# omahs/cess

Hardware: AMD Instinct MI355X
Metric: verified BLS12-381 sigs/sec (node) (higher is better)
Workload: dtype u32 (381-bit Montgomery, 14x28-bit limb products via v_mad_u64_u32)

## Files before the change

cess_amd/csrc/bls/pair_fe.hpp:

```cpp
#pragma once
#include "pair.hpp"

#if !defined(CESS_HOSTEMU)
namespace bls {

struct GlobPair {
  uint4* base;
  uint64_t stride;
  CESS_HD uint64_t at(int k, int q) const {
    const uint32_t l = lane_fresh();
    return (uint64_t)(6 * k + q + 3 * (l & 1u)) * stride + (l >> 1);
  }
  CESS_HD fph ld(int k) const {
    fph r;
#pragma unroll
    for (int q = 0; q < 3; q++) {
      const uint4 x = base[at(k, q)];
      r.v.v[4 * q] = x.x, r.v.v[4 * q + 1] = x.y, r.v.v[4 * q + 2] = x.z, r.v.v[4 * q + 3] = x.w;
    }
    return r;
  }
  CESS_HD void st(int k, const fph& a) const {
#pragma unroll
    for (int q = 0; q < 3; q++)
      base[at(k, q)] = make_uint4(a.v.v[4 * q], a.v.v[4 * q + 1], a.v.v[4 * q + 2], a.v.v[4 * q + 3]);
  }
  CESS_HD fp2 ld_full(int k) const {
    const uint32_t l = lane_fresh() >> 1;
    fp2 r;
#pragma unroll
    for (int q = 0; q < 6; q++) {
      const uint4 x = base[(uint64_t)(6 * k + q) * stride + l];
      fp& d = q < 3 ? r.c0 : r.c1;
      const int o = 4 * (q % 3);
      d.v[o] = x.x, d.v[o + 1] = x.y, d.v[o + 2] = x.z, d.v[o + 3] = x.w;
    }
    return r;
  }
  CESS_HD void st_full(int k, const fp2& a) const {
    const uint32_t l = lane_fresh() >> 1;
#pragma unroll
    for (int q = 0; q < 6; q++) {
      const fp& s = q < 3 ? a.c0 : a.c1;
      const int o = 4 * (q % 3);
      base[(uint64_t)(6 * k + q) * stride + l] = make_uint4(s.v[o], s.v[o + 1], s.v[o + 2], s.v[o + 3]);
    }
  }
};

template <class D, class S>
CESS_HD void pcopy12(const D& d, const S& s) {
#pragma unroll 1
  for (int k = 0; k < 6; k++) d.st(k, s.ld(k));
}
template <class S>
CESS_HD void pconj12(const S& f) {
#pragma unroll 1
  for (int k = 3; k < 6; k++) f.st(k, neg(f.ld(k)));
}
template <class S>
CESS_HD bool pis_one12(const S& f) {
  bool r = eq(f.ld(0).v, fph_one().v);
#pragma unroll 1
  for (int k = 1; k < 6; k++) r = r && is_zero(f.ld(k).v);
  return pair_and(r);
}
template <class A, class B>
CESS_HD bool pis_conj12(const A& a, const B& b) {
  bool r = true;
#pragma unroll 1
  for (int k = 0; k < 6; k++) r = r && eq(a.ld(k).v, k < 3 ? b.ld(k).v : neg(b.ld(k).v));
  return pair_and(r);
}

template <class LA>
CESS_HD fp6h pmul6_lr(LA&& a, const fp6h& b) {
#if CESS_PAIR_SB
  return pmul6_sb(a, b);
#endif
  const fph v0 = pmul(a(0), b.c0);
  CESS_MEMBAR();
  const fph v1 = pmul(a(1), b.c1);
  CESS_MEMBAR();
  const fph v2 = pmul(a(2), b.c2);
  CESS_MEMBAR();
  const fph c0 = add(mul_nr(sub(sub(pmul(add_nr(a(1), a(2)), add_nr(b.c1, b.c2)), v1), v2)), v0);
  CESS_MEMBAR();
  const fph c1 = add(sub(sub(pmul(add_nr(a(0), a(1)), add_nr(b.c0, b.c1)), v0), v1), mul_nr(v2));
  CESS_MEMBAR();
  const fph c2 = add(sub(sub(pmul(add_nr(a(0), a(2)), add_nr(b.c0, b.c2)), v0), v2), v1);
  return {c0, c1, c2};
}

#ifndef CESS_PAIR_FE_LOOP
#define CESS_PAIR_FE_LOOP 1
#endif
template <class S, class G>
CESS_HD void pmul12(const S& f, const G& g) {
#if CESS_PAIR_FE_LOOP
  fp6h t0;
#pragma unroll 1
  for (int it = 0; it < 3; it++) {
    fp6h b;
    if (it == 1) {
      b = add_nr(pld6(g, 0), pld6(g, 1));
    } else {
      b = pld6(g, it >> 1);
    }
    const fp6h r = pmul6_lr(
        [&](int j) {
          const int lo = it == 2 ? 3 : 0;
          const fph a = f.ld(lo + j);
          return it == 1 ? add_nr(a, f.ld(3 + j)) : a;
        },
        b);
    CESS_MEMBAR();
    if (it == 0) {
      t0 = r;
    } else if (it == 1) {
      pst6(f, 0, sub(r, t0));
    } else {
      pst6(f, 1, sub(pld6(f, 0), r));
      pst6(f, 0, add(t0, mul_v(r)));
    }
  }
#else
  fp6h t0;
  {
    const fp6h g0 = pld6(g, 0);
    t0 = pmul6_lr([&](int j) { return f.ld(j); }, g0);
  }
  CESS_MEMBAR();
  {
    fp6h gs;
    {
      const fp6h g0 = pld6(g, 0), g1 = pld6(g, 1);
      gs = add_nr(g0, g1);
    }
    const fp6h x = pmul6_lr([&](int j) { return add_nr(f.ld(j), f.ld(3 + j)); }, gs);
    CESS_MEMBAR();
    pst6(f, 0, sub(x, t0));
  }
  CESS_MEMBAR();
  fp6h t1;
  {
    const fp6h g1 = pld6(g, 1);
    t1 = pmul6_lr([&](int j) { return f.ld(3 + j); }, g1);
  }
  CESS_MEMBAR();
  pst6(f, 1, sub(pld6(f, 0), t1));
  pst6(f, 0, add(t0, mul_v(t1)));
#endif
}

template <class S>
CESS_HD fp6h psqr6(const S& f, int h) {
  const fp6h a = pld6(f, h);
  return pmul6_lr([&](int j) { return f.ld(3 * h + j); }, a);
}

template <class S>
CESS_HD void pinv12(const S& f) {
  fp6h ti;
  {
    fp6h t;
    {
      const fp6h s0 = psqr6(f, 0);
      CESS_MEMBAR();
      t = sub(s0, mul_v(psqr6(f, 1)));
    }
    CESS_MEMBAR();
    const fph c0 = sub(pmul(t.c0, t.c0), mul_nr(pmul(t.c1, t.c2)));
    CESS_MEMBAR();
    const fph c1 = sub(mul_nr(pmul(t.c2, t.c2)), pmul(t.c0, t.c1));
    CESS_MEMBAR();
    const fph c2 = sub(pmul(t.c1, t.c1), pmul(t.c0, t.c2));
    CESS_MEMBAR();
    const fph den = add(pmul(t.c0, c0), mul_nr(pdot2(t.c2, c1, t.c1, c2)));
    const fph di = pinv(den);
    CESS_MEMBAR();
    ti = {pmul(c0, di), pmul(c1, di), pmul(c2, di)};
  }
  CESS_MEMBAR();
  pst6(f, 0, pmul6_lr([&](int j) { return f.ld(j); }, ti));
  CESS_MEMBAR();
  const fp6h r1 = pmul6_lr([&](int j) { return f.ld(3 + j); }, ti);
  pst6(f, 1, {neg(r1.c0), neg(r1.c1), neg(r1.c2)});
}

CESS_HD fph pfrob_coeff(int k, int i) {
  const uint32_t hm = pair_hi_mask();
  fp r;
#pragma unroll
  for (int w = 0; w < 12; w++) r.v[w] = (c::FROB[k - 1][i][1][w] & hm) | (c::FROB[k - 1][i][0][w] & ~hm);
  return {r};
}
template <class S>
CESS_HD void pfrob12(const S& f, int k) {
#pragma unroll 1
  for (int s = 0; s < 6; s++) {
    const int i = (s % 3) * 2 + s / 3;
    fph y = f.ld(s);
    if (k & 1) y = conj(y);
    if (i) y = pmul(y, pfrob_coeff(k, i));
    f.st(s, y);
  }
}

CESS_HD void pfp4_square(fph& c0, fph& c1, const fph& a, const fph& b) {
  const fph t0 = pmul(a, b);
  CESS_MEMBAR();
  const fph t = pmul(add_nr(a, b), add_xi_nr(a, b));
  c0 = sub(sub(t, t0), mul_nr(t0));
  c1 = dbl(t0);
}
CESS_HD void pcyc_square_regs(fph (&z)[6], int n) {
#pragma unroll 1
  for (int r = 0; r < n; r++) {
    CESS_MEMBAR();
    fph t0, t1;
    pfp4_square(t0, t1, z[0], z[4]);
    z[0] = add(dbl(sub(t0, z[0])), t0);
    z[4] = add(dbl(add(t1, z[4])), t1);
    CESS_MEMBAR();
    fph t2, t3;
    pfp4_square(t0, t1, z[3], z[2]);
    CESS_MEMBAR();
    pfp4_square(t2, t3, z[1], z[5]);
    z[1] = add(dbl(sub(t0, z[1])), t0);
    z[5] = add(dbl(add(t1, z[5])), t1);
    const fph n3 = mul_nr(t3);
    z[3] = add(dbl(add(n3, z[3])), n3);
    z[2] = add(dbl(sub(t2, z[2])), t2);
  }
}
template <class S>
CESS_HD void pcyc_square_run(const S& f, int n) {
  fph z[6];
#pragma unroll
  for (int k = 0; k < 6; k++) z[k] = f.ld(k);
  pcyc_square_regs(z, n);
#pragma unroll
  for (int k = 0; k < 6; k++) f.st(k, z[k]);
}

CESS_HD void pkcyc_run(fph& z2, fph& z3, fph& z4, fph& z5, int n) {
#pragma unroll 1
  for (int r = 0; r < n; r++) {
    CESS_MEMBAR();
    fph u, v;
    {
      const fph b3 = pmul_scaled<3>(z4, z5);
      CESS_MEMBAR();
      const fph t3 = pmul_scaled<3>(add_nr(z4, z5), add_xi_nr(z4, z5));
      const fph nb3 = mul_nr(b3);
      u = sub(sub(t3, b3), nb3);
      v = dbl(nb3);
    }
    CESS_MEMBAR();
    {
      const fph b3 = pmul_scaled<3>(z2, z3);
      CESS_MEMBAR();
      const fph t3 = pmul_scaled<3>(add_nr(z2, z3), add_xi_nr(z2, z3));
      z4 = sub(sub(sub(t3, b3), mul_nr(b3)), dbl(z4));
      z5 = dbl(add(z5, b3));
    }
    CESS_MEMBAR();
    z2 = add(dbl(z2), v);
    z3 = sub(u, dbl(z3));
  }
}

CESS_HD fp2 xchg2(const fp2& a) { return {xchg(a.c0), xchg(a.c1)}; }

CESS_HD void ps_operands(const fp2& u, const fp2& w, bool hi, fp2& s, fp2& y) {
  uint32_t bn = 0, k0 = 0, k1 = 0, k2 = 0, k3 = 0;
#pragma unroll
  for (int i = 0; i < 12; i++) {
    const uint32_t z0 = hi ? u.c0.v[i] : w.c0.v[i], z1 = hi ? u.c1.v[i] : w.c1.v[i];
    const uint32_t nz1 = subc32(c::P2_RAW[i], z1, bn, &bn);
    s.c0.v[i] = addc32(u.c0.v[i], w.c0.v[i], k0, &k0);
    s.c1.v[i] = addc32(u.c1.v[i], w.c1.v[i], k1, &k1);
    y.c0.v[i] = addc32(s.c0.v[i], nz1, k2, &k2);
    y.c1.v[i] = addc32(s.c1.v[i], z0, k3, &k3);
  }
}
CESS_HD void pkcyc_run_ps(fp2& u, fp2& w, int n) {
  const bool hi = pair_hi_mask() != 0;
#pragma unroll 1
  for (int r = 0; r < n; r++) {
    CESS_MEMBAR();
    fp2 P, Q;
    {
      const fp2 b3 = mul_scaled<3>(u, w);
      CESS_MEMBAR();
      fp2 s, y;
      ps_operands(u, w, hi, s, y);
      const fp2 t3 = mul_scaled<3>(s, y);
      const fp2 nb3 = mul_nr(b3);
      P = sub(sub(t3, b3), nb3);
      Q = select(hi, b3, nb3);
    }
    CESS_MEMBAR();
    P = xchg2(P);
    Q = xchg2(Q);
    u = sub(P, dbl(u));
    w = dbl(add(w, Q));
  }
}

CESS_HD void pcyc_z1_frac(const fph& z2, const fph& z3, const fph& z4, const fph& z5, fph& num, fph& den) {
  if (is_zero(z2)) {
    num = dbl(pmul(z4, z5));
    den = z3;
  } else {
    num = sub(add(mul_nr(psqr(z5)), mul3(psqr(z4))), dbl(z3));
    den = dbl(dbl(z2));
  }
}
CESS_HD fph pcyc_z1_den(const fph& z2, const fph& z3) { return is_zero(z2) ? z3 : dbl(dbl(z2)); }
CESS_HD fph pcyc_z0(const fph& z1, const fph& z2, const fph& z3, const fph& z4, const fph& z5) {
  return add(mul_nr(add(dbl(psqr(z1)), pdot2(z2, z5, neg(mul3(z3)), z4))), fph_one());
}

template <class B, class XFn>
CESS_HD void pcyc_chain(const B& base, XFn&& X) {
  constexpr int ND = CESS_CHAIN_TAIL ? 3 : 6;
#ifndef CESS_PAIR_KCYC_PS
#define CESS_PAIR_KCYC_PS 1
#endif
#if CESS_PAIR_KCYC_PS
  {
    const bool hi = pair_hi_mask() != 0;
    const int ku = hi ? 2 : 1, kw = hi ? 3 : 5;
    fp2 u = base.ld_full(ku), w = base.ld_full(kw);
    int k = 0;
#pragma unroll 1
    for (int j = 0; j < ND; j++) {
      const int stop = j == 0 ? 16 : j == 1 ? 48 : j == 2 ? 57 : j == 3 ? 60 : j == 4 ? 62 : 63;
      pkcyc_run_ps(u, w, stop - k);
      k = stop;
      CESS_MEMBAR();
      const auto x = X(j);
      x.st_full(ku, u);
      x.st_full(kw, w);
    }
  }
#else
  {
    fph z4 = base.ld(1), z5 = base.ld(5), z2 = base.ld(3), z3 = base.ld(2);
    int k = 0;
#pragma unroll 1
    for (int j = 0; j < ND; j++) {
      const int stop = j == 0 ? 16 : j == 1 ? 48 : j == 2 ? 57 : j == 3 ? 60 : j == 4 ? 62 : 63;
      pkcyc_run(z2, z3, z4, z5, stop - k);
      k = stop;
      CESS_MEMBAR();
      const auto x = X(j);
      x.st(3, z2);
      x.st(2, z3);
      x.st(1, z4);
      x.st(5, z5);
    }
  }
#endif
  CESS_MEMBAR();
  bool degen = false;
  fph prod = fph_one();
#pragma unroll 1
  for (int j = 0; j < ND; j++) {
    const auto x = X(j);
    fph num, den;
    pcyc_z1_frac(x.ld(3), x.ld(2), x.ld(1), x.ld(5), num, den);
    const bool z = is_zero(den);
    degen = degen || z;
    x.st(4, num);
    x.st(0, prod);
    prod = pmul(prod, select(z, fph_one(), den));
    CESS_MEMBAR();
  }
  fph iv = pinv(prod);
#pragma unroll 1
  for (int j = ND - 1; j >= 0; j--) {
    const auto x = X(j);
    const fph den = pcyc_z1_den(x.ld(3), x.ld(2));
    const fph ivj = pmul(iv, x.ld(0));
    iv = pmul(iv, select(is_zero(den), fph_one(), den));
    CESS_MEMBAR();
    const fph z1 = pmul(x.ld(4), ivj);
    x.st(4, z1);
    CESS_MEMBAR();
    x.st(0, pcyc_z0(z1, x.ld(3), x.ld(2), x.ld(1), x.ld(5)));
    CESS_MEMBAR();
  }
  if (degen) {
    const auto w = X(5);
    pcopy12(w, base);
#pragma unroll 1
    for (int j = 0; j < 5; j++) {
      const int run = j == 0 ? 16 : j == 1 ? 32 : j == 2 ? 9 : j == 3 ? 3 : 2;
      pcyc_square_run(w, run);
      pcopy12(X(j), w);
    }
    pcyc_square_run(w, 1);
  }
#if CESS_CHAIN_TAIL
  else {
    fph z[6];
    {
      const auto x2 = X(2);
#pragma unroll
      for (int k = 0; k < 6; k++) z[k] = x2.ld(k);
    }
#pragma unroll 1
    for (int j = 3; j < 6; j++) {
      pcyc_square_regs(z, j == 3 ? 3 : j == 4 ? 2 : 1);
      CESS_MEMBAR();
      const auto x = X(j);
#pragma unroll
      for (int k = 0; k < 6; k++) x.st(k, z[k]);
    }
  }
#endif
}

template <class A, class SlotFn>
CESS_HD void final_exp_pair(const A& acc, const uint8_t (*prog)[2], SlotFn&& slot) {
#pragma unroll 1
  for (int pc = 0;; pc++) {
    const uint8_t op = prog[pc][0], arg = prog[pc][1];
    if (op == FE_END) break;
    switch (op) {
      case FE_LOAD: pcopy12(acc, slot(arg)); break;
      case FE_STORE: pcopy12(slot(arg), acc); break;
      case FE_MUL: pmul12(acc, slot(arg)); break;
      case FE_SQN: pcyc_square_run(acc, arg); break;
      case FE_CONJ: pconj12(acc); break;
      case FE_FROB: pfrob12(acc, arg); break;
      case FE_INV: pinv12(acc); break;
      case FE_CHAIN: pcyc_chain(slot(arg), [&](int j) { return slot(SL_X0 + j); }); break;
      default: break;
    }
    CESS_MEMBAR();
  }
}

}
#endif
```

cess_amd/csrc/bls/staged.hpp:

```cpp
#pragma once
#include "pairing.hpp"
#include "diag.hpp"

namespace bls {

#if !defined(CESS_HOSTEMU)
CESS_HD uint32_t lane_fresh() {
  uint32_t l;
  asm volatile("v_mbcnt_lo_u32_b32 %0, -1, 0\n\tv_mbcnt_hi_u32_b32 %0, -1, %0" : "=v"(l));
  return l;
}
CESS_HD uint32_t wave_first_thread() { return __builtin_amdgcn_readfirstlane(threadIdx.x & ~63u); }

struct LdsF12 {
  uint4 (*F)[256];
  uint32_t w0;
  CESS_HD fp2 ld(int k) const {
    const uint32_t t = w0 + lane_fresh();
    fp2 r;
#pragma unroll
    for (int q = 0; q < 6; q++) {
      uint4 x = F[6 * k + q][t];
      fp& d = q < 3 ? r.c0 : r.c1;
      const int o = 4 * (q % 3);
      d.v[o] = x.x, d.v[o + 1] = x.y, d.v[o + 2] = x.z, d.v[o + 3] = x.w;
    }
    return r;
  }
  CESS_HD void st(int k, const fp2& a) const {
    const uint32_t t = w0 + lane_fresh();
#pragma unroll
    for (int q = 0; q < 6; q++) {
      const fp& s = q < 3 ? a.c0 : a.c1;
      const int o = 4 * (q % 3);
      F[6 * k + q][t] = make_uint4(s.v[o], s.v[o + 1], s.v[o + 2], s.v[o + 3]);
    }
  }
};

struct GlobF12W {
  uint4* base;
  uint64_t stride;
  CESS_HD fp2 ld(int k) const {
    const uint32_t l = lane_fresh();
    fp2 r;
#pragma unroll
    for (int q = 0; q < 6; q++) {
      uint4 x = base[(uint64_t)(6 * k + q) * stride + l];
      fp& d = q < 3 ? r.c0 : r.c1;
      const int o = 4 * (q % 3);
      d.v[o] = x.x, d.v[o + 1] = x.y, d.v[o + 2] = x.z, d.v[o + 3] = x.w;
    }
    return r;
  }
  CESS_HD void st(int k, const fp2& a) const {
    const uint32_t l = lane_fresh();
#pragma unroll
    for (int q = 0; q < 6; q++) {
      const fp& s = q < 3 ? a.c0 : a.c1;
      const int o = 4 * (q % 3);
      const uint4 v = make_uint4(s.v[o], s.v[o + 1], s.v[o + 2], s.v[o + 3]);
      base[(uint64_t)(6 * k + q) * stride + l] = v;
    }
  }
};

struct GlobF12 {
  uint4* base;
  uint64_t stride;
  uint32_t i;
  CESS_HD fp2 ld(int k) const {
    fp2 r;
#pragma unroll
    for (int q = 0; q < 6; q++) {
      uint4 x = base[(uint64_t)(6 * k + q) * stride + i];
      fp& d = q < 3 ? r.c0 : r.c1;
      const int o = 4 * (q % 3);
      d.v[o] = x.x, d.v[o + 1] = x.y, d.v[o + 2] = x.z, d.v[o + 3] = x.w;
    }
    return r;
  }
  CESS_HD void st(int k, const fp2& a) const {
#pragma unroll
    for (int q = 0; q < 6; q++) {
      const fp& s = q < 3 ? a.c0 : a.c1;
      const int o = 4 * (q % 3);
      base[(uint64_t)(6 * k + q) * stride + i] = make_uint4(s.v[o], s.v[o + 1], s.v[o + 2], s.v[o + 3]);
    }
  }
};
#endif

struct ArrF12 {
  fp12* p;
  CESS_HD fp2 ld(int k) const { return (&p->c0.c0)[k]; }
  CESS_HD void st(int k, const fp2& a) const { (&p->c0.c0)[k] = a; }
};

template <class S>
CESS_HD fp6 ld6(const S& s, int h) {
  return {s.ld(3 * h), s.ld(3 * h + 1), s.ld(3 * h + 2)};
}
template <class S>
CESS_HD void st6(const S& s, int h, const fp6& a) {
  s.st(3 * h, a.c0);
  s.st(3 * h + 1, a.c1);
  s.st(3 * h + 2, a.c2);
}
template <class D, class S>
CESS_HD void copy12(const D& d, const S& s) {
#pragma unroll 1
  for (int k = 0; k < 6; k++) d.st(k, s.ld(k));
}
template <class S>
CESS_HD void set_one12(const S& s) {
  s.st(0, fp2_one());
#pragma unroll 1
  for (int k = 1; k < 6; k++) s.st(k, fp2_zero());
}
template <class S>
CESS_HD void conj12(const S& s) {
#pragma unroll 1
  for (int k = 3; k < 6; k++) s.st(k, neg(s.ld(k)));
}
template <class S>
CESS_HD bool is_one12(const S& s) {
  bool r = eq(s.ld(0), fp2_one());
#pragma unroll 1
  for (int k = 1; k < 6; k++) r = r && is_zero(s.ld(k));
  return r;
}

template <class A, class B>
CESS_HD bool is_conj12(const A& a, const B& b) {
  bool r = true;
#pragma unroll 1
  for (int k = 0; k < 6; k++) r = r && eq(a.ld(k), k < 3 ? b.ld(k) : neg(b.ld(k)));
  return r;
}

#ifndef CESS_SQR12_LOOP
#define CESS_SQR12_LOOP 0
#endif
#ifndef CESS_MUL014_LOOP
#define CESS_MUL014_LOOP 0
#endif
template <class S>
CESS_HD void sqr12(const S& f) {
#if CESS_SQR12_LOOP
  fp6 ab;
#pragma unroll 1
  for (int it = 0; it < 2; it++) {
    fp6 x, y;
    {
      const fp6 a0 = ld6(f, 0), a1 = ld6(f, 1);
      if (it) {
        x = add_nr(a0, a1);
        y = add_nr(a0, mul_v(a1));
      } else {
        x = a0;
        y = a1;
      }
    }
    const fp6 r = mul(x, y);
    CESS_MEMBAR();
    if (it) {
      st6(f, 0, sub(sub(r, ab), mul_v(ab)));
      st6(f, 1, dbl(ab));
    } else {
      ab = r;
    }
  }
#else
  fp6 ab;
  {
    fp6 a0 = ld6(f, 0), a1 = ld6(f, 1);
    ab = mul(a0, a1);
  }
  CESS_MEMBAR();
  fp6 x;
  {
    fp6 a0 = ld6(f, 0), a1 = ld6(f, 1);
    x = mul(add_nr(a0, a1), add_nr(a0, mul_v(a1)));
  }
  st6(f, 0, sub(sub(x, ab), mul_v(ab)));
  st6(f, 1, dbl(ab));
#endif
}

template <class S>
CESS_HD fp6 mul_by_01_dot(const S& f, int h, const fp2& b0, const fp2& b1, const fp2& xb1) {
  fp6 r;
  r.c0 = dot2(f.ld(3 * h), b0, f.ld(3 * h + 2), xb1);
  CESS_MEMBAR();
  r.c1 = dot2(f.ld(3 * h), b1, f.ld(3 * h + 1), b0);
  CESS_MEMBAR();
  r.c2 = dot2(f.ld(3 * h + 1), b1, f.ld(3 * h + 2), b0);
  return r;
}

template <class S>
CESS_HD void mul014(const S& f, const fp2& c0, const fp2& c1, const fp2& c4) {
#if CESS_MUL014_LOOP
  fp6 bb = mul_by_1(ld6(f, 1), c4);
  CESS_MEMBAR();
  fp6 aa;
  const fp2 d = add(c1, c4);
#pragma unroll 1
  for (int it = 0; it < 2; it++) {
    const fp2 b1 = it ? d : c1;
    const fp6 r = mul_by_01_dot(f, it, c0, b1, mul_nr(b1));
    CESS_MEMBAR();
    if (it) {
      st6(f, 1, sub(r, add(aa, bb)));
    } else {
      aa = r;
      {
        fp6 s = add(ld6(f, 0), ld6(f, 1));
        st6(f, 1, s);
      }
      st6(f, 0, add(mul_v(bb), aa));
    }
  }
#else
  fp6 bb = mul_by_1(ld6(f, 1), c4);
  CESS_MEMBAR();
  fp6 aa = mul_by_01_dot(f, 0, c0, c1, mul_nr(c1));
  CESS_MEMBAR();
  {
    fp6 s = add(ld6(f, 0), ld6(f, 1));
    st6(f, 1, s);
  }
  st6(f, 0, add(mul_v(bb), aa));
  fp6 u = add(aa, bb);
  CESS_MEMBAR();
  const fp2 d = add(c1, c4);
  fp6 t = mul_by_01_dot(f, 1, c0, d, mul_nr(d));
  st6(f, 1, sub(t, u));
#endif
}

CESS_HD fp6 mul_by_01_one(const fp6& a, const fp2& b1) {
#if CESS_MUL2
  fp2 p2, p0;
  mul2(a.c2, b1, a.c0, b1, p2, p0);
  return {add(a.c0, mul_nr(p2)), add(a.c1, p0), add(a.c2, mul(a.c1, b1))};
#else
  return {add(a.c0, mul_nr(mul(a.c2, b1))), add(a.c1, mul(a.c0, b1)), add(a.c2, mul(a.c1, b1))};
#endif
}

template <class S>
CESS_HD void mul014_one(const S& f, const fp2& c1, const fp2& c4) {
#if CESS_MUL014_LOOP
  fp6 bb = mul_by_1(ld6(f, 1), c4);
  CESS_MEMBAR();
  fp6 aa;
  const fp2 d = add(c1, c4);
#pragma unroll 1
  for (int it = 0; it < 2; it++) {
    const fp6 r = mul_by_01_one(ld6(f, it), it ? d : c1);
    CESS_MEMBAR();
    if (it) {
      st6(f, 1, sub(r, add(aa, bb)));
    } else {
      aa = r;
      {
        fp6 s = add(ld6(f, 0), ld6(f, 1));
        st6(f, 1, s);
      }
      st6(f, 0, add(mul_v(bb), aa));
    }
  }
#else
  fp6 bb = mul_by_1(ld6(f, 1), c4);
  CESS_MEMBAR();
  fp6 aa = mul_by_01_one(ld6(f, 0), c1);
  CESS_MEMBAR();
  {
    fp6 s = add(ld6(f, 0), ld6(f, 1));
    st6(f, 1, s);
  }
  st6(f, 0, add(mul_v(bb), aa));
  fp6 u = add(aa, bb);
  CESS_MEMBAR();
  fp6 t = mul_by_01_one(ld6(f, 1), add(c1, c4));
  st6(f, 1, sub(t, u));
#endif
}

template <class S, class G>
CESS_HD void mul12(const S& f, const G& g) {
  fp6 t0, t1;
  t0 = mul(ld6(f, 0), ld6(g, 0));
  CESS_MEMBAR();
  t1 = mul(ld6(f, 1), ld6(g, 1));
  CESS_MEMBAR();
  fp6 x = mul(add_nr(ld6(f, 0), ld6(f, 1)), add_nr(ld6(g, 0), ld6(g, 1)));
  st6(f, 1, sub(sub(x, t0), t1));
  st6(f, 0, add(t0, mul_v(t1)));
}

#ifndef CESS_FE_PF
#define CESS_FE_PF 0
#endif
template <class LA, class LB, class SK>
CESS_HD void mul6_stream(LA&& a, LB&& b, SK&& sink) {
#if CESS_FE_PF
  fp2 pa = a(0), pb = b(0);
  fp2 qa = a(1), qb = b(1);
  const fp2 v0 = mul(pa, pb);
  CESS_MEMBAR();
  pa = a(2), pb = b(2);
  const fp2 v1 = mul(qa, qb);
  CESS_MEMBAR();
  const fp2 v2 = mul(pa, pb);
  CESS_MEMBAR();
#else
  const fp2 v0 = mul(a(0), b(0));
  CESS_MEMBAR();
  const fp2 v1 = mul(a(1), b(1));
  CESS_MEMBAR();
  const fp2 v2 = mul(a(2), b(2));
  CESS_MEMBAR();
#endif
  sink(0, add(mul_nr(sub(sub(mul(add_nr(a(1), a(2)), add_nr(b(1), b(2))), v1), v2)), v0));
  CESS_MEMBAR();
  sink(1, add(sub(sub(mul(add_nr(a(0), a(1)), add_nr(b(0), b(1))), v0), v1), mul_nr(v2)));
  CESS_MEMBAR();
  sink(2, add(sub(sub(mul(add_nr(a(0), a(2)), add_nr(b(0), b(2))), v0), v2), v1));
  CESS_MEMBAR();
}

template <class D, class S, class G, class T>
CESS_HD void mul12_stream(const D& d, const S& f, const G& g, const T& t) {
  mul6_stream([&](int j) { return f.ld(j); }, [&](int j) { return g.ld(j); },
              [&](int j, const fp2& v) { t.st(j, v); });
  mul6_stream([&](int j) { return f.ld(3 + j); }, [&](int j) { return g.ld(3 + j); },
              [&](int j, const fp2& v) { d.st(3 + j, v); });
  d.st(0, add(t.ld(0), mul_nr(d.ld(5))));
  d.st(1, add(t.ld(1), d.ld(3)));
  d.st(2, add(t.ld(2), d.ld(4)));
  CESS_MEMBAR();
  mul6_stream([&](int j) { return add_nr(f.ld(j), f.ld(3 + j)); },
              [&](int j) { return add_nr(g.ld(j), g.ld(3 + j)); },
              [&](int j, const fp2& x) { d.st(3 + j, sub(sub(x, t.ld(j)), d.ld(3 + j))); });
}

#ifndef CESS_FE_APARK
#define CESS_FE_APARK 1
#endif
template <class D, class S, class G, class T, class P>
CESS_HD void mul12_stream_ap(const D& d, const S& f, const G& g, const T& t, const P& pk) {
#pragma unroll 1
  for (int j = 0; j < 3; j++) pk.st(j, f.ld(j));
  CESS_MEMBAR();
  mul6_stream([&](int j) { return pk.ld(j); }, [&](int j) { return g.ld(j); },
              [&](int j, const fp2& v) { t.st(j, v); });
  CESS_MEMBAR();
#pragma unroll 1
  for (int j = 0; j < 3; j++) pk.st(j, f.ld(3 + j));
  CESS_MEMBAR();
  mul6_stream([&](int j) { return pk.ld(j); }, [&](int j) { return g.ld(3 + j); },
              [&](int j, const fp2& v) { d.st(3 + j, v); });
  d.st(0, add(t.ld(0), mul_nr(d.ld(5))));
  d.st(1, add(t.ld(1), d.ld(3)));
  d.st(2, add(t.ld(2), d.ld(4)));
  CESS_MEMBAR();
#pragma unroll 1
  for (int j = 0; j < 3; j++) pk.st(j, add_nr(f.ld(j), f.ld(3 + j)));
  CESS_MEMBAR();
  mul6_stream([&](int j) { return pk.ld(j); }, [&](int j) { return add_nr(g.ld(j), g.ld(3 + j)); },
              [&](int j, const fp2& x) { d.st(3 + j, sub(sub(x, t.ld(j)), d.ld(3 + j))); });
}

template <class S>
CESS_HD void cycsq12(const S& f) {
  {
    fp2 z0 = f.ld(0), z1 = f.ld(4), t0, t1;
    fp4_square(t0, t1, z0, z1);
    f.st(0, add(dbl(sub(t0, z0)), t0));
    f.st(4, add(dbl(add(t1, z1)), t1));
  }
  CESS_MEMBAR();
  fp2 t0, t1, t2, t3;
  fp4_square(t0, t1, f.ld(3), f.ld(2));
  fp4_square(t2, t3, f.ld(1), f.ld(5));
  f.st(1, add(dbl(sub(t0, f.ld(1))), t0));
  f.st(5, add(dbl(add(t1, f.ld(5))), t1));
  fp2 n3 = mul_nr(t3);
  f.st(3, add(dbl(add(n3, f.ld(3))), n3));
  f.st(2, add(dbl(sub(t2, f.ld(2))), t2));
}

template <class S>
CESS_HD void frob12(const S& f, int k) {
#pragma unroll 1
  for (int s = 0; s < 6; s++) {
    const int i = (s % 3) * 2 + s / 3;
    fp2 y = f.ld(s);
    if (k & 1) y = conj(y);
    if (i) y = mul(y, frob_coeff(k, i));
    f.st(s, y);
  }
}

template <class S>
CESS_HD void inv12(const S& f) {
  fp6 t;
  {
    fp6 a0 = ld6(f, 0), a1 = ld6(f, 1);
    t = sub(sqr(a0), mul_v(sqr(a1)));
  }
  t = inv(t);
  CESS_MEMBAR();
  fp6 a0 = ld6(f, 0);
  st6(f, 0, mul(a0, t));
  fp6 a1 = ld6(f, 1);
  st6(f, 1, neg(mul(a1, t)));
}

template <class D, class S, class T>
CESS_HD void inv12_stream(const D& d, const S& f, const T& t) {
  mul6_stream([&](int j) { return f.ld(j); }, [&](int j) { return f.ld(j); }, [&](int j, const fp2& v) { d.st(j, v); });
  mul6_stream([&](int j) { return f.ld(3 + j); }, [&](int j) { return f.ld(3 + j); },
              [&](int j, const fp2& v) { d.st(3 + j, v); });
  t.st(0, sub(d.ld(0), mul_nr(d.ld(5))));
  t.st(1, sub(d.ld(1), d.ld(3)));
  t.st(2, sub(d.ld(2), d.ld(4)));
  CESS_MEMBAR();
  d.st(0, sub(sqr(t.ld(0)), mul_nr(mul(t.ld(1), t.ld(2)))));
  CESS_MEMBAR();
  d.st(1, sub(mul_nr(sqr(t.ld(2))), mul(t.ld(0), t.ld(1))));
  CESS_MEMBAR();
  d.st(2, sub(sqr(t.ld(1)), mul(t.ld(0), t.ld(2))));
  CESS_MEMBAR();
  const fp2 den = inv(add(mul(t.ld(0), d.ld(0)), mul_nr(add(mul(t.ld(2), d.ld(1)), mul(t.ld(1), d.ld(2))))));
  CESS_MEMBAR();
#pragma unroll 1
  for (int j = 0; j < 3; j++) t.st(j, mul(d.ld(j), den));
  CESS_MEMBAR();
  mul6_stream([&](int j) { return f.ld(j); }, [&](int j) { return t.ld(j); }, [&](int j, const fp2& v) { d.st(j, v); });
  mul6_stream([&](int j) { return f.ld(3 + j); }, [&](int j) { return t.ld(j); },
              [&](int j, const fp2& v) { d.st(3 + j, neg(v)); });
}

enum FeOp : uint8_t { FE_LOAD, FE_STORE, FE_MUL, FE_SQN, FE_CONJ, FE_FROB, FE_INV, FE_CHAIN, FE_END };
enum FeSlot : uint8_t { SL_F = 0, SL_M, SL_T0, SL_T1, SL_T3, SL_T4, SL_T5, SL_T6,
                        SL_X0, SL_X1, SL_X2, SL_X3, SL_X4, SL_X5, SL_TM, SL_N };

#define CESS_FE_CYCEXP(s) \
  {FE_CHAIN, s}, {FE_LOAD, SL_X5}, {FE_MUL, SL_X4}, {FE_MUL, SL_X3}, {FE_MUL, SL_X2}, {FE_MUL, SL_X1}, \
      {FE_MUL, SL_X0}, {FE_CONJ, 0}

#define CESS_FE_BODY                                                                                              \
  {FE_LOAD, SL_F}, {FE_CONJ, 0}, {FE_STORE, SL_T0}, {FE_LOAD, SL_F}, {FE_INV, 0}, {FE_MUL, SL_T0},                 \
      {FE_STORE, SL_T0}, {FE_FROB, 2}, {FE_MUL, SL_T0}, {FE_STORE, SL_M},                                          \
       {FE_SQN, 1}, {FE_CONJ, 0}, {FE_STORE, SL_T1},                                     \
       CESS_FE_CYCEXP(SL_M), {FE_STORE, SL_T3},                                                      \
       {FE_SQN, 1}, {FE_STORE, SL_T4},                                                          \
       {FE_LOAD, SL_T1}, {FE_MUL, SL_T3}, {FE_STORE, SL_T5},                                     \
       CESS_FE_CYCEXP(SL_T5), {FE_STORE, SL_T1},                                                    \
       CESS_FE_CYCEXP(SL_T1), {FE_STORE, SL_T0},                                                    \
       CESS_FE_CYCEXP(SL_T0), {FE_MUL, SL_T4}, {FE_STORE, SL_T6},                             \
       CESS_FE_CYCEXP(SL_T6), {FE_STORE, SL_T4},                                                    \
       {FE_LOAD, SL_T5}, {FE_CONJ, 0}, {FE_MUL, SL_M}, {FE_MUL, SL_T4},              \
      {FE_STORE, SL_T4},                                                                                           \
       {FE_LOAD, SL_T1}, {FE_MUL, SL_M}, {FE_FROB, 3}, {FE_STORE, SL_T1},                 \
       {FE_LOAD, SL_M}, {FE_CONJ, 0}, {FE_MUL, SL_T6}, {FE_FROB, 1},              \
      {FE_STORE, SL_T6},                                                                                           \
       {FE_LOAD, SL_T3}, {FE_MUL, SL_T0}, {FE_FROB, 2}, {FE_MUL, SL_T1},  \
      {FE_MUL, SL_T6}
#define CESS_FE_PROGRAM CESS_FE_BODY, {FE_MUL, SL_T4}, {FE_END, 0}
#define CESS_FE_PROGRAM_VERIFY CESS_FE_BODY, {FE_END, 0}

template <class A, class P>
CESS_HD void cyc_square_run(const A& acc, const P& pk, int n) {
  pk.st(0, acc.ld(0));
  pk.st(1, acc.ld(4));
  fp2 z2 = acc.ld(3), z3 = acc.ld(2);
#pragma unroll 1
  for (int r = 0; r < n; r++) {
    CESS_MEMBAR();
    {
      const fp2 a = pk.ld(0), b = pk.ld(1);
      fp2 t0, t1;
      fp4_square(t0, t1, a, b);
      pk.st(0, add(dbl(sub(t0, a)), t0));
      pk.st(1, add(dbl(add(t1, b)), t1));
    }
    CESS_MEMBAR();
    fp2 u0;
    {
      fp2 u1;
      fp4_square(u0, u1, acc.ld(1), acc.ld(5));
      pk.st(2, u1);
    }
    CESS_MEMBAR();
    {
      fp2 t0, t1;
      fp4_square(t0, t1, z2, z3);
      acc.st(1, add(dbl(sub(t0, acc.ld(1))), t0));
      acc.st(5, add(dbl(add(t1, acc.ld(5))), t1));
    }
    CESS_MEMBAR();
    const fp2 n3 = mul_nr(pk.ld(2));
    z2 = add(dbl(add(n3, z2)), n3);
    z3 = add(dbl(sub(u0, z3)), u0);
  }
  CESS_MEMBAR();
  acc.st(0, pk.ld(0));
  acc.st(4, pk.ld(1));
  acc.st(3, z2);
  acc.st(2, z3);
}

#ifndef CESS_KCYC_LOOP
#define CESS_KCYC_LOOP 0
#endif
template <class P>
CESS_HD void kcyc_run(const P& pk, fp2& z2, fp2& z3, int n) {
#if CESS_KCYC_LOOP
#pragma unroll 1
  for (int r = 0; r < n; r++) {
    fp2 u, v;
#pragma unroll 1
    for (int h = 0; h < 2; h++) {
      CESS_MEMBAR();
      fp2 x, y;
      if (h) {
        x = z2;
        y = z3;
      } else {
        x = pk.ld(0);
        y = pk.ld(1);
      }
      const fp2 b3 = mul_scaled<3>(x, y);
      CESS_MEMBAR();
      const fp2 t3 = mul_scaled<3>(add_nr(x, y), add_xi_nr(x, y));
      const fp2 nb3 = mul_nr(b3);
      const fp2 w = sub(sub(t3, b3), nb3);
      if (h) {
        pk.st(0, sub(w, dbl(pk.ld(0))));
        pk.st(1, dbl(add(pk.ld(1), b3)));
      } else {
        u = w;
        v = dbl(nb3);
      }
    }
    CESS_MEMBAR();
    z2 = add(dbl(z2), v);
    z3 = sub(u, dbl(z3));
  }
#else
#pragma unroll 1
  for (int r = 0; r < n; r++) {
    CESS_MEMBAR();
    fp2 u, v;
    {
      const fp2 b3 = mul_scaled<3>(pk.ld(0), pk.ld(1));
      CESS_MEMBAR();
      const fp2 t3 = mul_scaled<3>(add_nr(pk.ld(0), pk.ld(1)), add_xi_nr(pk.ld(0), pk.ld(1)));
      const fp2 nb3 = mul_nr(b3);
      u = sub(sub(t3, b3), nb3);
      v = dbl(nb3);
    }
    CESS_MEMBAR();
    {
      const fp2 b3 = mul_scaled<3>(z2, z3);
      CESS_MEMBAR();
      const fp2 t3 = mul_scaled<3>(add_nr(z2, z3), add_xi_nr(z2, z3));
      pk.st(0, sub(sub(sub(t3, b3), mul_nr(b3)), dbl(pk.ld(0))));
      pk.st(1, dbl(add(pk.ld(1), b3)));
    }
    CESS_MEMBAR();
    z2 = add(dbl(z2), v);
    z3 = sub(u, dbl(z3));
  }
#endif
}

CESS_HD void cyc_z1_frac(const fp2& z2, const fp2& z3, const fp2& z4, const fp2& z5, fp2& num, fp2& den) {
  num = sub(add(mul_nr(sqr(z5)), mul3(sqr(z4))), dbl(z3));
  den = dbl(dbl(z2));
  if (is_zero(z2)) {
    num = dbl(mul(z4, z5));
    den = z3;
  }
}
CESS_HD fp2 cyc_z1_den(const fp2& z2, const fp2& z3) { return is_zero(z2) ? z3 : dbl(dbl(z2)); }
CESS_HD fp2 cyc_z0(const fp2& z1, const fp2& z2, const fp2& z3, const fp2& z4, const fp2& z5) {
  return add(mul_nr(add(dbl(sqr(z1)), dot2(z2, z5, neg(mul3(z3)), z4))), fp2_one());
}

#ifndef CESS_CHAIN_TAIL
#define CESS_CHAIN_TAIL 1
#endif
template <class B, class XFn, class P, class DG = NoDiag>
CESS_HD void cyc_chain(const B& base, XFn&& X, const P& pk, DG* dg = nullptr) {
  constexpr int ND = CESS_CHAIN_TAIL ? 3 : 6;
  {
    pk.st(0, base.ld(1));
    pk.st(1, base.ld(5));
    fp2 z2 = base.ld(3), z3 = base.ld(2);
    int k = 0;
#pragma unroll 1
    for (int j = 0; j < ND; j++) {
      const int stop = j == 0 ? 16 : j == 1 ? 48 : j == 2 ? 57 : j == 3 ? 60 : j == 4 ? 62 : 63;
      if (dg) dg->template mark<0>();
      kcyc_run(pk, z2, z3, stop - k);
      if (dg) dg->template mark<3>();
      k = stop;
      CESS_MEMBAR();
      const auto x = X(j);
      x.st(3, z2);
      x.st(2, z3);
      x.st(1, pk.ld(0));
      x.st(5, pk.ld(1));
    }
  }
  CESS_MEMBAR();
  bool degen = false;
  fp2 prod = fp2_one();
#pragma unroll 1
  for (int j = 0; j < ND; j++) {
    const auto x = X(j);
    fp2 num, den;
    cyc_z1_frac(x.ld(3), x.ld(2), x.ld(1), x.ld(5), num, den);
    const bool z = is_zero(den);
    degen = degen || z;
    x.st(4, num);
    x.st(0, prod);
    prod = mul(prod, select(z, fp2_one(), den));
    CESS_MEMBAR();
  }
  fp2 iv = inv(prod);
#pragma unroll 1
  for (int j = ND - 1; j >= 0; j--) {
    const auto x = X(j);
    const fp2 den = cyc_z1_den(x.ld(3), x.ld(2));
    const fp2 ivj = mul(iv, x.ld(0));
    iv = mul(iv, select(is_zero(den), fp2_one(), den));
    CESS_MEMBAR();
    const fp2 z1 = mul(x.ld(4), ivj);
    x.st(4, z1);
    CESS_MEMBAR();
    x.st(0, cyc_z0(z1, x.ld(3), x.ld(2), x.ld(1), x.ld(5)));
    CESS_MEMBAR();
  }
  if (degen) {
    const auto w = X(5);
    copy12(w, base);
#pragma unroll 1
    for (int j = 0; j < 5; j++) {
      const int run = j == 0 ? 16 : j == 1 ? 32 : j == 2 ? 9 : j == 3 ? 3 : 2;
      cyc_square_run(w, pk, run);
      copy12(X(j), w);
    }
    cyc_square_run(w, pk, 1);
  }
#if CESS_CHAIN_TAIL
  else {
#pragma unroll 1
    for (int j = 3; j < 6; j++) {
      copy12(X(j), X(j - 1));
      cyc_square_run(X(j), pk, j == 3 ? 3 : j == 4 ? 2 : 1);
    }
  }
#endif
  if (dg) dg->template mark<4>();
}

template <class A, class SlotFn, class P, class DG = NoDiag>
CESS_HD int final_exp_staged(const A& acc0, const A& acc1, const uint8_t (*prog)[2], SlotFn&& slot, const P& pk,
                             DG* dg = nullptr) {
  int cur = 0;
#pragma unroll 1
  for (int pc = 0;; pc++) {
    const uint8_t op = prog[pc][0], arg = prog[pc][1];
    if (op == FE_END) break;
    const A& acc = cur ? acc1 : acc0;
    switch (op) {
      case FE_LOAD: copy12(acc, slot(arg)); break;
      case FE_STORE: copy12(slot(arg), acc); break;
      case FE_MUL:
#if CESS_FE_APARK
        mul12_stream_ap(cur ? acc0 : acc1, acc, slot(arg), slot(SL_TM), pk);
#else
        mul12_stream(cur ? acc0 : acc1, acc, slot(arg), pk);
#endif
        cur ^= 1;
        if (dg) dg->template mark<1>();
        break;
      case FE_SQN: cyc_square_run(acc, pk, arg); break;
      case FE_CONJ: conj12(acc); break;
      case FE_FROB: frob12(acc, arg); break;
      case FE_INV:
        inv12_stream(cur ? acc0 : acc1, acc, pk);
        cur ^= 1;
        if (dg) dg->template mark<2>();
        break;
      case FE_CHAIN: cyc_chain(slot(arg), [&](int j) { return slot(SL_X0 + j); }, pk, dg); break;
      default: break;
    }
    if (dg) dg->template mark<0>();
  }
  return cur;
}

template <class S, class Pt, class Src, class DG = NoDiag>
CESS_HD void miller_loop2_staged(const S& f, bool use0, bool use1, Pt&& pt, Src&& src, bool norm1 = false,
                                 DG* dg = nullptr) {
  set_one12(f);
  if (dg) dg->template mark<5>();
#pragma unroll 1
  for (int s = 0; s < N_COEFFS; s++) {
#pragma unroll 1
    for (int pair = 0; pair < 2; pair++) {
      const int pr = 1 - pair;
      if (!(pr ? use1 : use0)) continue;
      coeff3 k = src(pr, s);
      g1a p = pt(pr);
      fp2 c1 = mul_fp(k.c1, p.x), c4 = mul_fp(k.c0, p.y);
      if (dg) {
        if (pr) dg->template mark<0>(); else dg->template mark<2>();
      }
      if (pr && !norm1)
        mul014(f, k.c2, c1, c4);
      else
        mul014_one(f, c1, c4);
      CESS_MEMBAR();
      if (dg) {
        if (pr) dg->template mark<1>(); else dg->template mark<3>();
      }
    }
    if (square_after_step(s)) sqr12(f);
    CESS_MEMBAR();
    if (dg) dg->template mark<4>();
  }
  conj12(f);
  if (dg) dg->template mark<5>();
}

template <int NP, class S, class Pt, class Src>
CESS_HD void miller_loopn_staged(const S& f, uint32_t use, Pt&& pt, Src&& src) {
  set_one12(f);
#pragma unroll 1
  for (int s = 0; s < N_COEFFS; s++) {
#pragma unroll 1
    for (int j = 0; j < NP; j++) {
      if (!((use >> j) & 1u)) continue;
      const coeff3 k = src(j, s);
      const g1a p = pt(j);
      const fp2 c1 = mul_fp(k.c1, p.x), c4 = mul_fp(k.c0, p.y);
      mul014(f, k.c2, c1, c4);
      CESS_MEMBAR();
    }
    if (square_after_step(s)) sqr12(f);
    CESS_MEMBAR();
  }
  conj12(f);
}

}
```

cess_amd/csrc/k_final.hip:

```cpp
#include <hip/hip_runtime.h>
#include "soa.hpp"

using namespace bls;
using namespace cess;

__constant__ uint8_t kFeProgram[][2] = {CESS_FE_PROGRAM};
__constant__ uint8_t kFeProgramVerify[][2] = {CESS_FE_PROGRAM_VERIFY};

#define CESS_LB_F12 __launch_bounds__(256, 2)

#if defined(CESS_DIAG)
CESS_DIAG_TABLE(k_final)
#endif

__global__ CESS_LB_F12 void k_final(uint64_t n, uint8_t* __restrict__ code, uint4* __restrict__ fin,
                                    uint4* __restrict__ slots, uint64_t* __restrict__ bitmap,
                                    uint8_t* __restrict__ gt_out, uint64_t stride) {
  uint32_t i = blockIdx.x * blockDim.x + threadIdx.x;
  uint8_t c = CODE_SIG_LEN;
  if (i < n) {
    c = code[i];
    if (c == 0) {
#if defined(CESS_FE_L2PROBE)
      const uint32_t w0 = wave_first_thread();
#else
      const uint32_t w0 = blockIdx.x * blockDim.x + wave_first_thread();
#endif
      GlobF12W acc0{slots + (uint64_t)(SL_N - 1) * 36 * stride + w0, stride};
      GlobF12W acc1{slots + (uint64_t)SL_N * 36 * stride + w0, stride};
      __shared__ uint4 park[18][256];
      auto slot = [&](int s) {
        return GlobF12W{(s == SL_F ? fin : slots + (uint64_t)(s - 1) * 36 * stride) + w0, stride};
      };
#if defined(CESS_DIAG)
      Diag dg;
      dg.begin();
      Diag* dgp = &dg;
#else
      NoDiag* dgp = nullptr;
#endif
      if (gt_out || !is_one12(slot(SL_F))) {
        const int which = final_exp_staged(acc0, acc1, gt_out ? kFeProgram : kFeProgramVerify, slot,
                                           LdsF12{park, wave_first_thread()}, dgp);
        const GlobF12W acc = which ? acc1 : acc0;
        if (!(gt_out ? is_one12(acc) : is_conj12(acc, slot(SL_T4)))) c = CODE_PAIRING;
        if (gt_out) {
#pragma unroll 1
          for (int k = 0; k < 6; k++) {
            fp2 e = acc.ld(k);
            uint8_t b[48];
            raw_to_be48(from_mont(e.c0), b);
            for (int t = 0; t < 48; t++) gt_out[576 * (uint64_t)i + 96 * k + t] = b[t];
            raw_to_be48(from_mont(e.c1), b);
            for (int t = 0; t < 48; t++) gt_out[576 * (uint64_t)i + 96 * k + 48 + t] = b[t];
          }
        }
      }
#if defined(CESS_DIAG)
      dg.mark<5>();
      dg.end(cess_diag_tab);
#endif
      code[i] = c;
    }
  }
  uint64_t ball = __ballot(c == 0);
  if ((threadIdx.x & 63) == 0 && i < n) bitmap[i >> 6] = ball;
}
```

cess_amd/csrc/kernels.hpp:

```cpp
#pragma once
#include <stdint.h>

#ifndef CESS_MIN_WAVES
#define CESS_MIN_WAVES 1
#endif
#define CESS_LB __launch_bounds__(256, CESS_MIN_WAVES)

enum : uint8_t {
  CODE_OK = 0,
  CODE_SIG_LEN = 1,
  CODE_SIG_POINT = 2,
  CODE_PK_LEN = 3,
  CODE_PK_POINT = 4,
  CODE_PAIRING = 5,
};
enum : uint8_t { PRE_SIG_LEN_BAD = 1, PRE_PK_LEN_BAD = 2 };
enum : uint8_t { INF_SIG = 1, INF_PK = 2 };

#define CESS_W_G1 24u
#define CESS_W_G2 48u
#define CESS_W_COEFFS 4896u
#define CESS_W_FP12 144u
#define CESS_FE_SLOTS 16u

#define CESS_MSM_SEG_BUCKETS 4096u
#ifndef CESS_PAIR_THREADS
#define CESS_PAIR_THREADS 256
#endif
#ifndef CESS_RLCD_PER
#define CESS_RLCD_PER 4
#endif
#define CESS_MSM_MAX_SEGS 256u
struct MsmSegs {
  const uint32_t *grp, *pos, *plo, *phi, *tlo, *thi;
  uint32_t nparts, nterms;
};
#if defined(__HIPCC__)
__host__ __device__
#endif
inline uint32_t msm_chunk(uint32_t cnt) {
  const uint32_t c = (cnt + 31u) / 32u;
  return c > 64u ? c : 64u;
}
```

Measured before the change: 3.130 million.

## Shorten cyclotomic exponent chain and add verify-specific final-exp program

The compressed-squaring chain for exponentiation by |x| now stores only three checkpoints (16, 48, 57) instead of six. The remaining low bits of x are rebuilt in the program with plain cyclotomic squarings, conjugations and multiplies, which frees two global slots per thread and drops one batched decompression. The verify path gets its own final-exponentiation addition chain that reorders the hard-part steps and ends without the final multiply by T4. This reduces slot traffic and memory footprint at the cost of extra full Fp12 multiplications, and correctness depends on the new chain encoding the same exponent.

```diff
diff --git a/cess_amd/csrc/bls/pair_fe.hpp b/cess_amd/csrc/bls/pair_fe.hpp
--- a/cess_amd/csrc/bls/pair_fe.hpp
+++ b/cess_amd/csrc/bls/pair_fe.hpp
@@ -325,7 +325,7 @@
 
 template <class B, class XFn>
 CESS_HD void pcyc_chain(const B& base, XFn&& X) {
-  constexpr int ND = CESS_CHAIN_TAIL ? 3 : 6;
+  constexpr int ND = 3;
 #ifndef CESS_PAIR_KCYC_PS
 #define CESS_PAIR_KCYC_PS 1
 #endif
@@ -337,7 +337,7 @@
     int k = 0;
 #pragma unroll 1
     for (int j = 0; j < ND; j++) {
-      const int stop = j == 0 ? 16 : j == 1 ? 48 : j == 2 ? 57 : j == 3 ? 60 : j == 4 ? 62 : 63;
+      const int stop = j == 0 ? 16 : j == 1 ? 48 : 57;
       pkcyc_run_ps(u, w, stop - k);
       k = stop;
       CESS_MEMBAR();
@@ -352,7 +352,7 @@
     int k = 0;
 #pragma unroll 1
     for (int j = 0; j < ND; j++) {
-      const int stop = j == 0 ? 16 : j == 1 ? 48 : j == 2 ? 57 : j == 3 ? 60 : j == 4 ? 62 : 63;
+      const int stop = j == 0 ? 16 : j == 1 ? 48 : 57;
       pkcyc_run(z2, z3, z4, z5, stop - k);
       k = stop;
       CESS_MEMBAR();
@@ -394,34 +394,14 @@
     CESS_MEMBAR();
   }
   if (degen) {
-    const auto w = X(5);
+    const auto w = X(2);
     pcopy12(w, base);
 #pragma unroll 1
-    for (int j = 0; j < 5; j++) {
-      const int run = j == 0 ? 16 : j == 1 ? 32 : j == 2 ? 9 : j == 3 ? 3 : 2;
-      pcyc_square_run(w, run);
-      pcopy12(X(j), w);
-    }
-    pcyc_square_run(w, 1);
-  }
-#if CESS_CHAIN_TAIL
-  else {
-    fph z[6];
-    {
-      const auto x2 = X(2);
-#pragma unroll
-      for (int k = 0; k < 6; k++) z[k] = x2.ld(k);
-    }
-#pragma unroll 1
-    for (int j = 3; j < 6; j++) {
-      pcyc_square_regs(z, j == 3 ? 3 : j == 4 ? 2 : 1);
-      CESS_MEMBAR();
-      const auto x = X(j);
-#pragma unroll
-      for (int k = 0; k < 6; k++) x.st(k, z[k]);
-    }
-  }
-#endif
+    for (int j = 0; j < ND; j++) {
+      pcyc_square_run(w, j == 0 ? 16 : j == 1 ? 32 : 9);
+      if (j < ND - 1) pcopy12(X(j), w);
+    }
+  }
 }
 
 template <class A, class SlotFn>
diff --git a/cess_amd/csrc/bls/staged.hpp b/cess_amd/csrc/bls/staged.hpp
--- a/cess_amd/csrc/bls/staged.hpp
+++ b/cess_amd/csrc/bls/staged.hpp
@@ -447,15 +447,19 @@
 
 enum FeOp : uint8_t { FE_LOAD, FE_STORE, FE_MUL, FE_SQN, FE_CONJ, FE_FROB, FE_INV, FE_CHAIN, FE_END };
 enum FeSlot : uint8_t { SL_F = 0, SL_M, SL_T0, SL_T1, SL_T3, SL_T4, SL_T5, SL_T6,
-                        SL_X0, SL_X1, SL_X2, SL_X3, SL_X4, SL_X5, SL_TM, SL_N };
-
-#define CESS_FE_CYCEXP(s) \
-  {FE_CHAIN, s}, {FE_LOAD, SL_X5}, {FE_MUL, SL_X4}, {FE_MUL, SL_X3}, {FE_MUL, SL_X2}, {FE_MUL, SL_X1}, \
-      {FE_MUL, SL_X0}, {FE_CONJ, 0}
+                        SL_X0, SL_X1, SL_X2, SL_XT, SL_TM, SL_N };
+
+#define CESS_FE_CYCEXP_ABS(s)                                                                                      \
+  {FE_CHAIN, s}, {FE_LOAD, SL_X2}, {FE_SQN, 3}, {FE_CONJ, 0}, {FE_MUL, SL_X2}, {FE_STORE, SL_XT}, {FE_SQN, 4},     \
+      {FE_CONJ, 0}, {FE_MUL, SL_XT}, {FE_MUL, SL_X1}, {FE_MUL, SL_X0}
+#define CESS_FE_CYCEXP(s) CESS_FE_CYCEXP_ABS(s), {FE_CONJ, 0}
+
+#define CESS_FE_EASY                                                                                              \
+  {FE_LOAD, SL_F}, {FE_CONJ, 0}, {FE_STORE, SL_T0}, {FE_LOAD, SL_F}, {FE_INV, 0}, {FE_MUL, SL_T0},                 \
+      {FE_STORE, SL_T0}, {FE_FROB, 2}, {FE_MUL, SL_T0}, {FE_STORE, SL_M}
 
 #define CESS_FE_BODY                                                                                              \
-  {FE_LOAD, SL_F}, {FE_CONJ, 0}, {FE_STORE, SL_T0}, {FE_LOAD, SL_F}, {FE_INV, 0}, {FE_MUL, SL_T0},                 \
-      {FE_STORE, SL_T0}, {FE_FROB, 2}, {FE_MUL, SL_T0}, {FE_STORE, SL_M},                                          \
+  CESS_FE_EASY,                                                                                                    \
        {FE_SQN, 1}, {FE_CONJ, 0}, {FE_STORE, SL_T1},                                     \
        CESS_FE_CYCEXP(SL_M), {FE_STORE, SL_T3},                                                      \
        {FE_SQN, 1}, {FE_STORE, SL_T4},                                                          \
@@ -472,7 +476,17 @@
        {FE_LOAD, SL_T3}, {FE_MUL, SL_T0}, {FE_FROB, 2}, {FE_MUL, SL_T1},  \
       {FE_MUL, SL_T6}
 #define CESS_FE_PROGRAM CESS_FE_BODY, {FE_MUL, SL_T4}, {FE_END, 0}
-#define CESS_FE_PROGRAM_VERIFY CESS_FE_BODY, {FE_END, 0}
+
+#define CESS_FE_PROGRAM_VERIFY                                                                                    \
+  CESS_FE_EASY,  {FE_SQN, 1}, {FE_STORE, SL_T4},                                                          \
+       CESS_FE_CYCEXP_ABS(SL_M), {FE_MUL, SL_M}, {FE_CONJ, 0}, {FE_STORE, SL_T0},                          \
+       CESS_FE_CYCEXP_ABS(SL_T0), {FE_MUL, SL_T0}, {FE_CONJ, 0}, {FE_STORE, SL_T1},                        \
+       {FE_FROB, 1}, {FE_STORE, SL_T3},                                                             \
+       CESS_FE_CYCEXP(SL_T1), {FE_MUL, SL_T3}, {FE_STORE, SL_T0},                                          \
+       {FE_FROB, 2}, {FE_STORE, SL_T3},                                                             \
+       CESS_FE_CYCEXP(SL_T0), {FE_STORE, SL_T1},                                                        \
+       CESS_FE_CYCEXP_ABS(SL_T1), {FE_MUL, SL_T0}, {FE_CONJ, 0}, {FE_MUL, SL_T3},                          \
+       {FE_MUL, SL_M}, {FE_END, 0}
 
 template <class A, class P>
 CESS_HD void cyc_square_run(const A& acc, const P& pk, int n) {
@@ -593,12 +607,9 @@
   return add(mul_nr(add(dbl(sqr(z1)), dot2(z2, z5, neg(mul3(z3)), z4))), fp2_one());
 }
 
-#ifndef CESS_CHAIN_TAIL
-#define CESS_CHAIN_TAIL 1
-#endif
 template <class B, class XFn, class P, class DG = NoDiag>
 CESS_HD void cyc_chain(const B& base, XFn&& X, const P& pk, DG* dg = nullptr) {
-  constexpr int ND = CESS_CHAIN_TAIL ? 3 : 6;
+  constexpr int ND = 3;
   {
     pk.st(0, base.ld(1));
     pk.st(1, base.ld(5));
@@ -606,7 +617,7 @@
     int k = 0;
 #pragma unroll 1
     for (int j = 0; j < ND; j++) {
-      const int stop = j == 0 ? 16 : j == 1 ? 48 : j == 2 ? 57 : j == 3 ? 60 : j == 4 ? 62 : 63;
+      const int stop = j == 0 ? 16 : j == 1 ? 48 : 57;
       if (dg) dg->template mark<0>();
       kcyc_run(pk, z2, z3, stop - k);
       if (dg) dg->template mark<3>();
@@ -649,25 +660,14 @@
     CESS_MEMBAR();
   }
   if (degen) {
-    const auto w = X(5);
+    const auto w = X(2);
     copy12(w, base);
 #pragma unroll 1
-    for (int j = 0; j < 5; j++) {
-      const int run = j == 0 ? 16 : j == 1 ? 32 : j == 2 ? 9 : j == 3 ? 3 : 2;
-      cyc_square_run(w, pk, run);
-      copy12(X(j), w);
-    }
-    cyc_square_run(w, pk, 1);
-  }
-#if CESS_CHAIN_TAIL
-  else {
-#pragma unroll 1
-    for (int j = 3; j < 6; j++) {
-      copy12(X(j), X(j - 1));
-      cyc_square_run(X(j), pk, j == 3 ? 3 : j == 4 ? 2 : 1);
-    }
-  }
-#endif
+    for (int j = 0; j < ND; j++) {
+      cyc_square_run(w, pk, j == 0 ? 16 : j == 1 ? 32 : 9);
+      if (j < ND - 1) copy12(X(j), w);
+    }
+  }
   if (dg) dg->template mark<4>();
 }
 
diff --git a/cess_amd/csrc/k_final.hip b/cess_amd/csrc/k_final.hip
--- a/cess_amd/csrc/k_final.hip
+++ b/cess_amd/csrc/k_final.hip
@@ -6,6 +6,7 @@
 
 __constant__ uint8_t kFeProgram[][2] = {CESS_FE_PROGRAM};
 __constant__ uint8_t kFeProgramVerify[][2] = {CESS_FE_PROGRAM_VERIFY};
+static_assert(CESS_FE_SLOTS == SL_N + 1, "host slot allocation: SL_M .. SL_TM and two accumulators");
 
 #define CESS_LB_F12 __launch_bounds__(256, 2)
 
diff --git a/cess_amd/csrc/kernels.hpp b/cess_amd/csrc/kernels.hpp
--- a/cess_amd/csrc/kernels.hpp
+++ b/cess_amd/csrc/kernels.hpp
@@ -21,7 +21,7 @@
 #define CESS_W_G2 48u
 #define CESS_W_COEFFS 4896u
 #define CESS_W_FP12 144u
-#define CESS_FE_SLOTS 16u
+#define CESS_FE_SLOTS 14u
 
 #define CESS_MSM_SEG_BUCKETS 4096u
 #ifndef CESS_PAIR_THREADS
```

After: 3.217 million, median of 6. 1.03x the previous value.
